# Zehong-Ma/MagCache

Measured on NVIDIA H100. Metric: denoising_steps_per_sec, higher is better.
Workload: dtype bf16

## Files before the change

magcache_b200/csrc/attn_wgmma.cu:

```cuda
#include <cstdlib>

#include "common.cuh"
#include "ptx.cuh"
#include "tma_host.cuh"

#ifndef MC_ATTN_EMU_DEFAULT
#define MC_ATTN_EMU_DEFAULT 0
#endif

namespace mc {

constexpr int kHD = 128;
constexpr int kLongMinLk = 1024;

struct AttnParams {
  int Lq, Lk, heads;
  int q_blocks, full_units, tail_units, tail_split;
  float* part_o;
  float2* part_ml;
  float scale_log2;
  __nv_bfloat16* out;
  int64_t ldo;
  int tile_rot;
  const uint32_t* seg_flags;
  const uint32_t* seg_epoch;
  int seg_rows;
};

struct WorkItem {
  int q_block, head;
  int split, nsplit;
  int tail_unit;
};

__device__ __forceinline__ WorkItem work_item(const AttnParams& p) {
  WorkItem w;
  int c = blockIdx.x, unit;
  if (c < p.full_units) {
    unit = c, w.split = 0, w.nsplit = 1, w.tail_unit = 0;
  } else {
    c -= p.full_units;
    w.tail_unit = c / p.tail_split;
    w.split = c - w.tail_unit * p.tail_split;
    w.nsplit = p.tail_split;
    unit = p.full_units + w.tail_unit;
  }
  w.head = unit / p.q_blocks;
  w.q_block = unit - w.head * p.q_blocks;
  return w;
}

template <uint32_t EMU_MASK>
__device__ __forceinline__ float exp2_sel(float x, int group) {
  return ((EMU_MASK >> (group & 7)) & 1u) ? ptx::ex2_emul(x) : ptx::ex2_approx(x);
}

__device__ __forceinline__ void wait_segments(const AttnParams& p, int row0, int rows) {
  if (p.seg_flags == nullptr) return;
  const uint32_t want = *reinterpret_cast<const volatile uint32_t*>(p.seg_epoch);
  const int last = min(row0 + rows, p.Lk) - 1;
  const int s0 = row0 / p.seg_rows, s1 = last / p.seg_rows;
  for (int s = s0; s <= s1; ++s) {
    const uint32_t* f = p.seg_flags + s;
    const long long t0 = clock64();
    for (;;) {
      uint32_t v;
      asm volatile("ld.acquire.sys.global.u32 %0, [%1];" : "=r"(v) : "l"(f) : "memory");
      if (static_cast<int32_t>(v - want) >= 0) break;
      __nanosleep(100);
      if (clock64() - t0 > MC_MBAR_TIMEOUT_CYCLES) {
        MC_DIAG("attention: key segment %d never arrived (flag %u, epoch %u)\n", s, v, want);
        __trap();
      }
    }
  }
  asm volatile("fence.proxy.async;" ::: "memory");
}

namespace ak {
constexpr int kBQ = 128;
constexpr int kQBytes = kBQ * kHD * 2;
constexpr int kThreads = 384;
constexpr int kProducerRegs = 24, kConsumerRegs = 240;
template <int BKV>
struct Layout {
  static constexpr int kKBytes = BKV * kHD * 2;
  static constexpr int kVBytes = BKV * kHD * 2;
  static constexpr int kOffK = kQBytes;
  static constexpr int kOffV = kOffK + 2 * kKBytes;
  static constexpr int kOffBar = kOffV + 2 * kVBytes;
  static constexpr int kSmem = kOffBar + 128;
};
}

template <int BKV, uint32_t EMU_MASK>
__global__ void __launch_bounds__(ak::kThreads, 1)
    attn_kernel(const __grid_constant__ CUtensorMap tmap_q, const __grid_constant__ CUtensorMap tmap_k,
                const __grid_constant__ CUtensorMap tmap_v, const AttnParams p) {
  using namespace ak;
  using L = Layout<BKV>;
  extern __shared__ __align__(1024) uint8_t smem[];
  uint64_t* bars = reinterpret_cast<uint64_t*>(smem + L::kOffBar);
  uint64_t* q_full = bars + 0;
  uint64_t* k_full = bars + 1;
  uint64_t* k_empty = bars + 3;
  uint64_t* v_full = bars + 5;
  uint64_t* v_empty = bars + 7;

  const int warp = threadIdx.x >> 5, lane = threadIdx.x & 31;
  const WorkItem wi = work_item(p);
  const int q0 = wi.q_block * kBQ;
  const int head = wi.head;
  const int total_tiles = (p.Lk + BKV - 1) / BKV;
  const int per_split = (total_tiles + wi.nsplit - 1) / wi.nsplit;
  const int t0 = wi.split * per_split;
  const int n_tiles = min(per_split, total_tiles - t0);
  auto tile_of = [&](int j) {
    int t = p.tile_rot + t0 + j;
    return t >= total_tiles ? t - total_tiles : t;
  };

  if (threadIdx.x == 0) {
    if ((ptx::smem_u32(smem) & 1023u) != 0) {
      MC_DIAG("attn_kernel: dynamic smem base not 1024-aligned\n");
      __trap();
    }
    ptx::prefetch_tmap(&tmap_q);
    ptx::prefetch_tmap(&tmap_k);
    ptx::prefetch_tmap(&tmap_v);
    ptx::mbar_init(q_full, 1);
    for (int s = 0; s < 2; ++s) {
      ptx::mbar_init(&k_full[s], 1);
      ptx::mbar_init(&k_empty[s], 8);
      ptx::mbar_init(&v_full[s], 1);
      ptx::mbar_init(&v_empty[s], 8);
    }
    ptx::fence_mbar_init();
  }
  __syncthreads();

  if (warp < 4) {
    ptx::setmaxnreg_dec<kProducerRegs>();
    if (warp == 0) {
      if (ptx::elect_one()) {
        ptx::mbar_expect_tx(q_full, kQBytes);
        ptx::tma_load_2d(smem, &tmap_q, q_full, head * kHD, q0);
        ptx::tma_load_2d(smem + kQBytes / 2, &tmap_q, q_full, head * kHD + 64, q0);
      }
      __syncwarp();
      for (int j = 0; j < n_tiles; ++j) {
        const int s = j & 1;
        const uint32_t ph = (j >> 1) & 1;
        const int kv0 = tile_of(j) * BKV;
        if (p.seg_flags != nullptr) {
          if (lane == 0) wait_segments(p, kv0, BKV);
          __syncwarp();
        }
        ptx::mbar_wait(&k_empty[s], ph ^ 1);
        if (ptx::elect_one()) {
          ptx::mbar_expect_tx(&k_full[s], L::kKBytes);
          ptx::tma_load_2d(smem + L::kOffK + s * L::kKBytes, &tmap_k, &k_full[s], head * kHD, kv0);
          ptx::tma_load_2d(smem + L::kOffK + s * L::kKBytes + L::kKBytes / 2, &tmap_k, &k_full[s], head * kHD + 64, kv0);
        }
        __syncwarp();
        ptx::mbar_wait(&v_empty[s], ph ^ 1);
        if (ptx::elect_one()) {
          ptx::mbar_expect_tx(&v_full[s], L::kVBytes);
          ptx::tma_load_2d(smem + L::kOffV + s * L::kVBytes, &tmap_v, &v_full[s], head * kHD, kv0);
          ptx::tma_load_2d(smem + L::kOffV + s * L::kVBytes + L::kVBytes / 2, &tmap_v, &v_full[s], head * kHD + 64, kv0);
        }
        __syncwarp();
      }
    }
  } else {
    ptx::setmaxnreg_inc<kConsumerRegs>();
    const int wg = (warp >> 2) - 1;
    const int r = wg * 64 + (warp & 3) * 16 + (lane >> 2);
    const int cq = 2 * (lane & 3);
    const uint32_t q_base = ptx::smem_u32(smem) + wg * (64 * 128);
    const uint32_t k_base = ptx::smem_u32(smem + L::kOffK), v_base = ptx::smem_u32(smem + L::kOffV);
    int j_ragged = -1;
    if (p.Lk % BKV != 0) {
      int jr = total_tiles - 1 - p.tile_rot - t0;
      if (jr < 0) jr += total_tiles;
      if (jr < n_tiles) j_ragged = jr;
    }
    float o[kHD / 2];
#pragma unroll
    for (int i = 0; i < kHD / 2; ++i) o[i] = 0.f;
    float m0 = -INFINITY, m1 = -INFINITY, l0 = 0.f, l1 = 0.f;
    bool timed_out = false;
    ptx::mbar_wait_or_flag(q_full, 0, timed_out);

    constexpr uint32_t kTurnThreads = 256;
    const uint32_t bar_own = 1 + wg, bar_other = 2 - wg;
    auto turn_begin = [&] { ptx::named_bar_sync(bar_own, kTurnThreads); };
    auto turn_end = [&] { ptx::named_bar_arrive(bar_other, kTurnThreads); };
    if (wg == 0) ptx::named_bar_arrive(bar_own, kTurnThreads);

    float sc[BKV / 2];
    uint32_t pa[BKV / 16][4];
    const int valid = p.Lk - (total_tiles - 1) * BKV;
    auto issue_s = [&](int j) {
      const int s = j & 1;
      ptx::wgmma_fence();
#pragma unroll
      for (int kk = 0; kk < kHD / 16; ++kk) {
        const uint64_t da = ptx::gmma_desc_sw128_kmajor(q_base + (kk >> 2) * (kQBytes / 2)) + 2 * (kk & 3);
        const uint64_t db = ptx::gmma_desc_sw128_kmajor(k_base + s * L::kKBytes + (kk >> 2) * (L::kKBytes / 2)) + 2 * (kk & 3);
        if constexpr (BKV == 128) {
          ptx::wgmma_m64n128k16_ss(sc, da, db, kk != 0 ? 1u : 0u);
        } else {
          ptx::wgmma_m64n64k16_ss(sc, da, db, kk != 0 ? 1u : 0u);
        }
      }
      ptx::wgmma_commit();
    };
    auto issue_pv = [&](int j) {
      const int s = j & 1;
      ptx::fence_regs(o);
      ptx::wgmma_fence();
      const uint64_t dv = ptx::gmma_desc_sw128_mnmajor(v_base + s * L::kVBytes, BKV * 128);
#pragma unroll
      for (int kk = 0; kk < BKV / 16; ++kk)
        ptx::wgmma_m64n128k16_rs_tb(o, pa[kk], dv + static_cast<uint64_t>(kk * (2048 / 16)), 1u);
      ptx::wgmma_commit();
    };
    auto softmax = [&](int j, float& f0, float& f1) {
      ptx::fence_regs(sc);
      __syncwarp();
      if (lane == 0) ptx::mbar_arrive(&k_empty[j & 1]);
      if (j == j_ragged) {
#pragma unroll
        for (int i = 0; i < BKV / 8; ++i)
#pragma unroll
          for (int e = 0; e < 4; ++e)
            if (8 * i + cq + (e & 1) >= valid) sc[4 * i + e] = -INFINITY;
      }
      float mx0 = -INFINITY, mx1 = -INFINITY;
#pragma unroll
      for (int i = 0; i < BKV / 8; ++i) {
        mx0 = fmaxf(mx0, fmaxf(sc[4 * i], sc[4 * i + 1]));
        mx1 = fmaxf(mx1, fmaxf(sc[4 * i + 2], sc[4 * i + 3]));
      }
#pragma unroll
      for (int off = 1; off <= 2; off <<= 1) {
        mx0 = fmaxf(mx0, __shfl_xor_sync(0xffffffffu, mx0, off));
        mx1 = fmaxf(mx1, __shfl_xor_sync(0xffffffffu, mx1, off));
      }
      const float mn0 = fmaxf(m0, mx0 * p.scale_log2), mn1 = fmaxf(m1, mx1 * p.scale_log2);
      f0 = ptx::ex2_approx(m0 - mn0), f1 = ptx::ex2_approx(m1 - mn1);
      m0 = mn0, m1 = mn1;
      l0 *= f0, l1 *= f1;
#pragma unroll
      for (int i = 0; i < BKV / 8; ++i) {
        sc[4 * i] = exp2_sel<EMU_MASK>(fmaf(sc[4 * i], p.scale_log2, -m0), i);
        sc[4 * i + 1] = exp2_sel<EMU_MASK>(fmaf(sc[4 * i + 1], p.scale_log2, -m0), i);
        sc[4 * i + 2] = exp2_sel<EMU_MASK>(fmaf(sc[4 * i + 2], p.scale_log2, -m1), i);
        sc[4 * i + 3] = exp2_sel<EMU_MASK>(fmaf(sc[4 * i + 3], p.scale_log2, -m1), i);
        l0 += sc[4 * i] + sc[4 * i + 1];
        l1 += sc[4 * i + 2] + sc[4 * i + 3];
      }
    };
    auto pack_p = [&] {
#pragma unroll
      for (int i = 0; i < BKV / 8; ++i) {
        pa[i >> 1][(i & 1) * 2] = pack_bf16x2(sc[4 * i], sc[4 * i + 1]);
        pa[i >> 1][(i & 1) * 2 + 1] = pack_bf16x2(sc[4 * i + 2], sc[4 * i + 3]);
      }
    };
    auto release_v = [&](int j) {
      ptx::fence_regs(o);
      __syncwarp();
      if (lane == 0) ptx::mbar_arrive(&v_empty[j & 1]);
    };
    auto rescale_o = [&](float f0, float f1) {
#pragma unroll
      for (int i = 0; i < kHD / 8; ++i) {
        o[4 * i] *= f0, o[4 * i + 1] *= f0;
        o[4 * i + 2] *= f1, o[4 * i + 3] *= f1;
      }
    };
    {
      ptx::mbar_wait_or_flag(&k_full[0], 0, timed_out);
      turn_begin();
      issue_s(0);
      turn_end();
      ptx::wgmma_wait<0>();
      float f0, f1;
      softmax(0, f0, f1);
      rescale_o(f0, f1);
      pack_p();
    }
    for (int j = 1; j < n_tiles; ++j) {
      ptx::mbar_wait_or_flag(&k_full[j & 1], (j >> 1) & 1, timed_out);
      ptx::mbar_wait_or_flag(&v_full[(j - 1) & 1], ((j - 1) >> 1) & 1, timed_out);
      turn_begin();
      issue_s(j);
      issue_pv(j - 1);
      turn_end();
      ptx::wgmma_wait<1>();
      float f0, f1;
      softmax(j, f0, f1);
      ptx::wgmma_wait<0>();
      release_v(j - 1);
      rescale_o(f0, f1);
      pack_p();
    }
    {
      const int j = n_tiles - 1;
      ptx::mbar_wait_or_flag(&v_full[j & 1], (j >> 1) & 1, timed_out);
      turn_begin();
      issue_pv(j);
      if (wg == 0) turn_end();
      ptx::wgmma_wait<0>();
      release_v(j);
    }
    if (timed_out) __trap();

#pragma unroll
    for (int off = 1; off <= 2; off <<= 1) {
      l0 += __shfl_xor_sync(0xffffffffu, l0, off);
      l1 += __shfl_xor_sync(0xffffffffu, l1, off);
    }
    const bool partial = wi.nsplit > 1;
#pragma unroll
    for (int h = 0; h < 2; ++h) {
      const float inv_l = 1.0f / (h ? l1 : l0);
      const int rt = r + 8 * h;
      const int row = q0 + rt;
      if (row >= p.Lq) continue;
      if (partial) {
        const int64_t prow = (static_cast<int64_t>(wi.split) * p.tail_units + wi.tail_unit) * kBQ + rt;
        if ((lane & 3) == 0) p.part_ml[prow] = make_float2(h ? m1 : m0, h ? l1 : l0);
        float* dst = p.part_o + prow * kHD + cq;
#pragma unroll
        for (int i = 0; i < kHD / 8; ++i)
          *reinterpret_cast<float2*>(dst + 8 * i) = make_float2(o[4 * i + 2 * h] * inv_l, o[4 * i + 2 * h + 1] * inv_l);
      } else {
        __nv_bfloat16* dst = p.out + static_cast<int64_t>(row) * p.ldo + head * kHD + cq;
#pragma unroll
        for (int i = 0; i < kHD / 8; ++i)
          *reinterpret_cast<uint32_t*>(dst + 8 * i) = pack_bf16x2(o[4 * i + 2 * h] * inv_l, o[4 * i + 2 * h + 1] * inv_l);
      }
    }
  }
}

__global__ void __launch_bounds__(256) attn_combine_kernel(const float* __restrict__ part_o, const float2* __restrict__ part_ml, int nsplit,
                                                           int tail_units, int full_units, int q_blocks, int rows_per_cta, int Lq,
                                                           __nv_bfloat16* __restrict__ out, int64_t ldo) {
  constexpr int kGroups = kHD / 8;
  const int64_t total = static_cast<int64_t>(tail_units) * rows_per_cta * kGroups;
  const int64_t split_stride = static_cast<int64_t>(tail_units) * rows_per_cta;
  for (int64_t i = static_cast<int64_t>(blockIdx.x) * blockDim.x + threadIdx.x; i < total; i += static_cast<int64_t>(gridDim.x) * blockDim.x) {
    const int64_t prow = i / kGroups;
    const int g = static_cast<int>(i - prow * kGroups);
    const int tu = static_cast<int>(prow / rows_per_cta), r = static_cast<int>(prow - static_cast<int64_t>(tu) * rows_per_cta);
    const int unit = full_units + tu;
    const int head = unit / q_blocks, row = (unit - head * q_blocks) * rows_per_cta + r;
    if (row >= Lq) continue;
    float mmax = -INFINITY;
    for (int s = 0; s < nsplit; ++s) mmax = fmaxf(mmax, part_ml[s * split_stride + prow].x);
    float acc[8] = {0.f, 0.f, 0.f, 0.f, 0.f, 0.f, 0.f, 0.f};
    float wsum = 0.f;
    for (int s = 0; s < nsplit; ++s) {
      const float2 ml = part_ml[s * split_stride + prow];
      const float w = ml.y * ptx::ex2_approx(ml.x - mmax);
      wsum += w;
      float v[8];
      ptx::ld_nc_v8_f32(part_o + (s * split_stride + prow) * kHD + g * 8, v);
#pragma unroll
      for (int j = 0; j < 8; ++j) acc[j] = fmaf(w, v[j], acc[j]);
    }
    const float inv = 1.0f / wsum;
#pragma unroll
    for (int j = 0; j < 8; ++j) acc[j] *= inv;
    *reinterpret_cast<uint4*>(out + static_cast<int64_t>(row) * ldo + head * kHD + g * 8) = pack_bf16x8(acc);
  }
}

struct AttnPlan {
  bool long_kernel;
  int q_blocks, kv_tile, total_tiles, rows_per_cta;
  int full_units, tail_units, tail_split;
  size_t ws_bytes;
  int grid() const { return full_units + tail_units * tail_split; }
};

static int env_int(const char* name, int lo, int hi, int dflt) {
  const char* e = getenv(name);
  if (!e || !*e) return dflt;
  const int v = atoi(e);
  return (v < lo || v > hi) ? dflt : v;
}

static AttnPlan plan_attention(int Lq, int Lk, int heads, bool need_long = false) {
  AttnPlan pl;
  const int forced_splits = env_int("MC_ATTN_SPLITS", 1, 16, 0);
  const int kernel_sel = env_int("MC_ATTN_KERNEL", 0, 2, 0);
  pl.long_kernel = need_long || kernel_sel == 2 || (kernel_sel == 0 && Lk >= kLongMinLk);
  pl.rows_per_cta = ak::kBQ;
  pl.kv_tile = pl.long_kernel ? 128 : 64;
  pl.q_blocks = (Lq + pl.rows_per_cta - 1) / pl.rows_per_cta;
  pl.total_tiles = (Lk + pl.kv_tile - 1) / pl.kv_tile;
  const int64_t units = static_cast<int64_t>(pl.q_blocks) * heads;
  const int slots = num_sms();
  const int min_tiles_per_split = pl.long_kernel ? 4 : 8;
  int full = static_cast<int>(units), tail = 0, split = 1;
  if (forced_splits > 0) {
    if (forced_splits > 1) full = 0, tail = static_cast<int>(units), split = forced_splits;
  } else {
    const int rem = static_cast<int>(units % slots);
    const int by_tiles = pl.total_tiles / min_tiles_per_split;
    int f = rem > 0 ? slots / rem : 1;
    if (f > 8) f = 8;
    if (f > by_tiles) f = by_tiles;
    if (f >= 2) full = static_cast<int>(units) - rem, tail = rem, split = f;
  }
  if (split > pl.total_tiles) split = pl.total_tiles;
  if (split > 1) {
    const int per = (pl.total_tiles + split - 1) / split;
    split = (pl.total_tiles + per - 1) / per;
  }
  if (split <= 1) full = static_cast<int>(units), tail = 0, split = 1;
  pl.full_units = full, pl.tail_units = tail, pl.tail_split = split;
  pl.ws_bytes = tail > 0 ? static_cast<size_t>(split) * tail * pl.rows_per_cta * (kHD * sizeof(float) + sizeof(float2)) : 0;
  return pl;
}

}

extern "C" int32_t mc_attn_workspace_bytes(int32_t Lq, int32_t Lk, int32_t heads, int64_t* bytes_out) {
  MC_CHECK_ARG(bytes_out != nullptr && Lq >= 1 && Lk >= 1 && heads >= 1, "mc_attn_workspace_bytes: bad arguments");
  const size_t a = mc::plan_attention(Lq, Lk, heads, false).ws_bytes, b = mc::plan_attention(Lq, Lk, heads, true).ws_bytes;
  *bytes_out = static_cast<int64_t>(a > b ? a : b);
  return MC_OK;
}

extern "C" int32_t mc_attn_fwd_ex(const void* q, int64_t ldq, const void* k, int64_t ldk, const void* v, int64_t ldv, void* out,
                                  int64_t ldo, int32_t Lq, int32_t Lk, int32_t heads, float scale, void* workspace,
                                  int64_t workspace_bytes, int32_t first_key_row, const uint32_t* seg_flags, const uint32_t* seg_epoch,
                                  int32_t seg_rows, void* stream) {
  MC_CHECK_ARG(q && k && v && out, "mc_attn_fwd: null pointer");
  MC_CHECK_ARG(Lq >= 1 && Lk >= 1 && heads >= 1, "mc_attn_fwd: Lq=%d Lk=%d heads=%d", Lq, Lk, heads);
  const int64_t width = static_cast<int64_t>(heads) * mc::kHD;
  MC_CHECK_ARG(ldq >= width && ldk >= width && ldo >= width && ldv >= width, "mc_attn_fwd: leading dimensions too small");
  MC_CHECK_ARG(ldq % 8 == 0 && ldk % 8 == 0 && ldv % 8 == 0 && ldo % 8 == 0, "mc_attn_fwd: leading dimensions must be multiples of 8");
  MC_CHECK_ARG(mc::aligned16(q) && mc::aligned16(k) && mc::aligned16(v) && mc::aligned16(out), "mc_attn_fwd: pointers must be 16-byte aligned");
  MC_CHECK_ARG(first_key_row >= 0 && first_key_row < Lk, "mc_attn_fwd: first_key_row=%d outside [0, %d)", first_key_row, Lk);
  MC_CHECK_ARG(seg_flags == nullptr || (seg_rows >= 1 && seg_epoch != nullptr), "mc_attn_fwd: seg_rows=%d / null epoch", seg_rows);
  const mc::AttnPlan pl = mc::plan_attention(Lq, Lk, heads, first_key_row != 0 || seg_flags != nullptr);
  MC_CHECK_ARG(static_cast<int64_t>(pl.q_blocks) * heads * 8 < INT32_MAX, "mc_attn_fwd: grid too large");
  if (pl.tail_units > 0) {
    MC_CHECK_ARG(workspace != nullptr && workspace_bytes >= static_cast<int64_t>(pl.ws_bytes) && (reinterpret_cast<uintptr_t>(workspace) & 31u) == 0,
                 "mc_attn_fwd: split-KV needs a 32-byte aligned workspace of %lld bytes (mc_attn_workspace_bytes), got %lld",
                 static_cast<long long>(pl.ws_bytes), static_cast<long long>(workspace_bytes));
  }
  const int q_box = mc::ak::kBQ;
  CUtensorMap tq, tk, tv;
  int32_t rc = mc::make_tmap_bf16_2d(&tq, q, static_cast<uint64_t>(Lq), static_cast<uint64_t>(width), static_cast<uint64_t>(ldq), q_box, 64);
  if (rc) return rc;
  rc = mc::make_tmap_bf16_2d(&tk, k, static_cast<uint64_t>(Lk), static_cast<uint64_t>(width), static_cast<uint64_t>(ldk), pl.kv_tile, 64);
  if (rc) return rc;
  rc = mc::make_tmap_bf16_2d(&tv, v, static_cast<uint64_t>(Lk), static_cast<uint64_t>(width), static_cast<uint64_t>(ldv), pl.kv_tile, 64);
  if (rc) return rc;

  float* part_o = static_cast<float*>(workspace);
  const size_t part_rows = static_cast<size_t>(pl.tail_split) * pl.tail_units * pl.rows_per_cta;
  float2* part_ml = pl.tail_units > 0 ? reinterpret_cast<float2*>(part_o + part_rows * mc::kHD) : nullptr;
  mc::AttnParams p{};
  p.Lq = Lq, p.Lk = Lk, p.heads = heads;
  p.q_blocks = pl.q_blocks, p.full_units = pl.full_units, p.tail_units = pl.tail_units, p.tail_split = pl.tail_split;
  p.part_o = pl.tail_units > 0 ? part_o : nullptr, p.part_ml = part_ml;
  p.scale_log2 = scale * 1.4426950408889634f;
  p.out = static_cast<__nv_bfloat16*>(out), p.ldo = ldo;
  p.tile_rot = ((first_key_row + pl.kv_tile - 1) / pl.kv_tile) % pl.total_tiles;
  p.seg_flags = seg_flags, p.seg_epoch = seg_epoch, p.seg_rows = seg_rows > 0 ? seg_rows : Lk;

  dim3 grid(pl.grid(), 1, 1);
  cudaStream_t st = static_cast<cudaStream_t>(stream);
  if (pl.long_kernel) {
    static mc::PerDeviceOnce once[4];
    const int emu = mc::env_int("MC_ATTN_EMU", 0, 4, MC_ATTN_EMU_DEFAULT);
#define MC_LAUNCH_LONG(MASK, IDX)                                                                                                    \
  do {                                                                                                                               \
    rc = mc::set_max_smem_once(mc::attn_kernel<128, MASK>, mc::ak::Layout<128>::kSmem, once[IDX], "cudaFuncSetAttribute(attn smem)"); \
    if (rc) return rc;                                                                                                               \
    mc::attn_kernel<128, MASK><<<grid, mc::ak::kThreads, mc::ak::Layout<128>::kSmem, st>>>(tq, tk, tv, p);                           \
  } while (0)
    switch (emu) {
      case 2: MC_LAUNCH_LONG(0x88u, 1); break;
      case 3: MC_LAUNCH_LONG(0x92u, 2); break;
      case 4: MC_LAUNCH_LONG(0xAAu, 3); break;
      default: MC_LAUNCH_LONG(0x00u, 0); break;
    }
#undef MC_LAUNCH_LONG
  } else {
    static mc::PerDeviceOnce once;
    rc = mc::set_max_smem_once(mc::attn_kernel<64, 0u>, mc::ak::Layout<64>::kSmem, once, "cudaFuncSetAttribute(attn smem)");
    if (rc) return rc;
    mc::attn_kernel<64, 0u><<<grid, mc::ak::kThreads, mc::ak::Layout<64>::kSmem, st>>>(tq, tk, tv, p);
  }
  MC_CHECK_LAUNCH("attn_kernel launch");
  if (pl.tail_units > 0) {
    const int64_t total = static_cast<int64_t>(pl.tail_units) * pl.rows_per_cta * (mc::kHD / 8);
    const int64_t want = (total + 255) / 256, cap = static_cast<int64_t>(mc::num_sms()) * 8;
    mc::attn_combine_kernel<<<static_cast<int>(want < cap ? want : cap), 256, 0, st>>>(
        p.part_o, p.part_ml, pl.tail_split, pl.tail_units, pl.full_units, pl.q_blocks, pl.rows_per_cta, Lq, static_cast<__nv_bfloat16*>(out), ldo);
    MC_CHECK_LAUNCH("attn_combine_kernel launch");
  }
  return MC_OK;
}

extern "C" int32_t mc_attn_fwd(const void* q, int64_t ldq, const void* k, int64_t ldk, const void* v, int64_t ldv, void* out,
                               int64_t ldo, int32_t Lq, int32_t Lk, int32_t heads, float scale, void* workspace,
                               int64_t workspace_bytes, void* stream) {
  return mc_attn_fwd_ex(q, ldq, k, ldk, v, ldv, out, ldo, Lq, Lk, heads, scale, workspace, workspace_bytes, 0, nullptr, nullptr, 0, stream);
}
```

Before: 1.661.

## Pair attention CTAs in 2-CTA clusters sharing K/V tiles via TMA multicast

```diff
diff --git a/magcache_b200/csrc/attn_wgmma.cu b/magcache_b200/csrc/attn_wgmma.cu
--- a/magcache_b200/csrc/attn_wgmma.cu
+++ b/magcache_b200/csrc/attn_wgmma.cu
@@ -33,16 +33,20 @@
   int tail_unit;
 };
 
+template <bool PAIR>
 __device__ __forceinline__ WorkItem work_item(const AttnParams& p) {
   WorkItem w;
-  int c = blockIdx.x, unit;
-  if (c < p.full_units) {
-    unit = c, w.split = 0, w.nsplit = 1, w.tail_unit = 0;
+  constexpr int kW = PAIR ? 2 : 1;
+  const int rank = PAIR ? static_cast<int>(ptx::cluster_ctarank()) : 0;
+  int c = PAIR ? static_cast<int>(blockIdx.x >> 1) : static_cast<int>(blockIdx.x), unit;
+  if (c < p.full_units / kW) {
+    unit = kW * c + rank, w.split = 0, w.nsplit = 1, w.tail_unit = 0;
   } else {
-    c -= p.full_units;
-    w.tail_unit = c / p.tail_split;
-    w.split = c - w.tail_unit * p.tail_split;
+    c -= p.full_units / kW;
+    const int item = c / p.tail_split;
+    w.split = c - item * p.tail_split;
     w.nsplit = p.tail_split;
+    w.tail_unit = kW * item + rank;
     unit = p.full_units + w.tail_unit;
   }
   w.head = unit / p.q_blocks;
@@ -82,6 +86,7 @@
 constexpr int kQBytes = kBQ * kHD * 2;
 constexpr int kThreads = 384;
 constexpr int kProducerRegs = 24, kConsumerRegs = 240;
+constexpr int kPairCluster = 2;
 template <int BKV>
 struct Layout {
   static constexpr int kKBytes = BKV * kHD * 2;
@@ -93,12 +98,14 @@
 };
 }
 
-template <int BKV, uint32_t EMU_MASK>
+template <int BKV, uint32_t EMU_MASK, bool PAIR>
 __global__ void __launch_bounds__(ak::kThreads, 1)
     attn_kernel(const __grid_constant__ CUtensorMap tmap_q, const __grid_constant__ CUtensorMap tmap_k,
                 const __grid_constant__ CUtensorMap tmap_v, const AttnParams p) {
   using namespace ak;
   using L = Layout<BKV>;
+  static_assert(!PAIR || BKV == 128, "only the 128-key kernel is paired");
+  constexpr uint32_t kCtas = PAIR ? kPairCluster : 1;
   extern __shared__ __align__(1024) uint8_t smem[];
   uint64_t* bars = reinterpret_cast<uint64_t*>(smem + L::kOffBar);
   uint64_t* q_full = bars + 0;
@@ -108,7 +115,7 @@
   uint64_t* v_empty = bars + 7;
 
   const int warp = threadIdx.x >> 5, lane = threadIdx.x & 31;
-  const WorkItem wi = work_item(p);
+  const WorkItem wi = work_item<PAIR>(p);
   const int q0 = wi.q_block * kBQ;
   const int head = wi.head;
   const int total_tiles = (p.Lk + BKV - 1) / BKV;
@@ -131,13 +138,18 @@
     ptx::mbar_init(q_full, 1);
     for (int s = 0; s < 2; ++s) {
       ptx::mbar_init(&k_full[s], 1);
-      ptx::mbar_init(&k_empty[s], 8);
+      ptx::mbar_init(&k_empty[s], 8 * kCtas);
       ptx::mbar_init(&v_full[s], 1);
-      ptx::mbar_init(&v_empty[s], 8);
+      ptx::mbar_init(&v_empty[s], 8 * kCtas);
     }
     ptx::fence_mbar_init();
   }
-  __syncthreads();
+  if constexpr (PAIR) {
+    ptx::cluster_arrive();
+    ptx::cluster_wait();
+  } else {
+    __syncthreads();
+  }
 
   if (warp < 4) {
     ptx::setmaxnreg_dec<kProducerRegs>();
@@ -148,26 +160,38 @@
         ptx::tma_load_2d(smem + kQBytes / 2, &tmap_q, q_full, head * kHD + 64, q0);
       }
       __syncwarp();
+      const uint32_t rank = PAIR ? ptx::cluster_ctarank() : 0u;
       for (int j = 0; j < n_tiles; ++j) {
         const int s = j & 1;
         const uint32_t ph = (j >> 1) & 1;
         const int kv0 = tile_of(j) * BKV;
+        const int row0 = kv0 + static_cast<int>(rank) * (BKV / kCtas);
+        const uint32_t part = rank * (L::kKBytes / 2 / kCtas);
+        auto load = [&](uint8_t* dst, const CUtensorMap* tmap, uint64_t* bar, int c0) {
+          if constexpr (PAIR) {
+            ptx::tma_load_2d_multicast(dst, tmap, bar, c0, row0, static_cast<uint16_t>((1u << kCtas) - 1));
+          } else {
+            ptx::tma_load_2d(dst, tmap, bar, c0, row0);
+          }
+        };
         if (p.seg_flags != nullptr) {
-          if (lane == 0) wait_segments(p, kv0, BKV);
+          if (lane == 0) wait_segments(p, row0, BKV / kCtas);
           __syncwarp();
         }
         ptx::mbar_wait(&k_empty[s], ph ^ 1);
         if (ptx::elect_one()) {
+          uint8_t* dst = smem + L::kOffK + s * L::kKBytes + part;
           ptx::mbar_expect_tx(&k_full[s], L::kKBytes);
-          ptx::tma_load_2d(smem + L::kOffK + s * L::kKBytes, &tmap_k, &k_full[s], head * kHD, kv0);
-          ptx::tma_load_2d(smem + L::kOffK + s * L::kKBytes + L::kKBytes / 2, &tmap_k, &k_full[s], head * kHD + 64, kv0);
+          load(dst, &tmap_k, &k_full[s], head * kHD);
+          load(dst + L::kKBytes / 2, &tmap_k, &k_full[s], head * kHD + 64);
         }
         __syncwarp();
         ptx::mbar_wait(&v_empty[s], ph ^ 1);
         if (ptx::elect_one()) {
+          uint8_t* dst = smem + L::kOffV + s * L::kVBytes + part;
           ptx::mbar_expect_tx(&v_full[s], L::kVBytes);
-          ptx::tma_load_2d(smem + L::kOffV + s * L::kVBytes, &tmap_v, &v_full[s], head * kHD, kv0);
-          ptx::tma_load_2d(smem + L::kOffV + s * L::kVBytes + L::kVBytes / 2, &tmap_v, &v_full[s], head * kHD + 64, kv0);
+          load(dst, &tmap_v, &v_full[s], head * kHD);
+          load(dst + L::kVBytes / 2, &tmap_v, &v_full[s], head * kHD + 64);
         }
         __syncwarp();
       }
@@ -226,10 +250,18 @@
         ptx::wgmma_m64n128k16_rs_tb(o, pa[kk], dv + static_cast<uint64_t>(kk * (2048 / 16)), 1u);
       ptx::wgmma_commit();
     };
+    auto release = [&](uint64_t* bar) {
+      if (lane != 0) return;
+      if constexpr (PAIR) {
+        for (uint32_t c = 0; c < kCtas; ++c) ptx::mbar_arrive_cluster(bar, c);
+      } else {
+        ptx::mbar_arrive(bar);
+      }
+    };
     auto softmax = [&](int j, float& f0, float& f1) {
       ptx::fence_regs(sc);
       __syncwarp();
-      if (lane == 0) ptx::mbar_arrive(&k_empty[j & 1]);
+      release(&k_empty[j & 1]);
       if (j == j_ragged) {
 #pragma unroll
         for (int i = 0; i < BKV / 8; ++i)
@@ -272,9 +304,10 @@
     auto release_v = [&](int j) {
       ptx::fence_regs(o);
       __syncwarp();
-      if (lane == 0) ptx::mbar_arrive(&v_empty[j & 1]);
+      release(&v_empty[j & 1]);
     };
     auto rescale_o = [&](float f0, float f1) {
+      if (!__any_sync(0xffffffffu, f0 != 1.f || f1 != 1.f)) return;
 #pragma unroll
       for (int i = 0; i < kHD / 8; ++i) {
         o[4 * i] *= f0, o[4 * i + 1] *= f0;
@@ -289,7 +322,6 @@
       ptx::wgmma_wait<0>();
       float f0, f1;
       softmax(0, f0, f1);
-      rescale_o(f0, f1);
       pack_p();
     }
     for (int j = 1; j < n_tiles; ++j) {
@@ -344,6 +376,10 @@
           *reinterpret_cast<uint32_t*>(dst + 8 * i) = pack_bf16x2(o[4 * i + 2 * h] * inv_l, o[4 * i + 2 * h + 1] * inv_l);
       }
     }
+  }
+  if constexpr (PAIR) {
+    ptx::cluster_arrive();
+    ptx::cluster_wait();
   }
 }
 
@@ -381,7 +417,7 @@
 }
 
 struct AttnPlan {
-  bool long_kernel;
+  bool long_kernel, paired;
   int q_blocks, kv_tile, total_tiles, rows_per_cta;
   int full_units, tail_units, tail_split;
   size_t ws_bytes;
@@ -395,28 +431,79 @@
   return (v < lo || v > hi) ? dflt : v;
 }
 
-static AttnPlan plan_attention(int Lq, int Lk, int heads, bool need_long = false) {
+static PerDeviceOnce g_attn_smem_once[2][4][2];
+
+template <uint32_t MASK>
+static int emu_index() {
+  return MASK == 0x88u ? 1 : MASK == 0x92u ? 2 : MASK == 0xAAu ? 3 : 0;
+}
+template <int BKV, uint32_t MASK, bool PAIR>
+static int32_t attn_set_smem() {
+  return set_max_smem_once(attn_kernel<BKV, MASK, PAIR>, ak::Layout<BKV>::kSmem, g_attn_smem_once[BKV == 128][emu_index<MASK>()][PAIR],
+                           "cudaFuncSetAttribute(attn smem)");
+}
+
+static int32_t attn_pair_clusters(int* out) {
+  static int cached[kMaxDevices] = {};
+  const int d = current_device();
+  if (cached[d] > 0) {
+    *out = cached[d];
+    return MC_OK;
+  }
+  int devices = 0;
+  if (cudaGetDeviceCount(&devices) != cudaSuccess || devices < 1) {
+    cudaGetLastError();
+    *out = num_sms() / ak::kPairCluster;
+    return MC_OK;
+  }
+  int32_t rc = attn_set_smem<128, 0u, true>();
+  if (rc) return rc;
+  cudaLaunchAttribute attr[1];
+  attr[0].id = cudaLaunchAttributeClusterDimension;
+  attr[0].val.clusterDim.x = ak::kPairCluster, attr[0].val.clusterDim.y = 1, attr[0].val.clusterDim.z = 1;
+  cudaLaunchConfig_t cfg = {};
+  cfg.gridDim = dim3(ak::kPairCluster * num_sms(), 1, 1);
+  cfg.blockDim = dim3(ak::kThreads, 1, 1);
+  cfg.dynamicSmemBytes = ak::Layout<128>::kSmem;
+  cfg.attrs = attr, cfg.numAttrs = 1;
+  int n = 0;
+  const cudaError_t e = cudaOccupancyMaxActiveClusters(&n, attn_kernel<128, 0u, true>, &cfg);
+  if (e != cudaSuccess) return cuda_fail(e, "cudaOccupancyMaxActiveClusters(attn)");
+  if (n < 1) {
+    set_error("attn_kernel: no cluster of %d CTAs with %d B of shared memory fits on this device", ak::kPairCluster, ak::Layout<128>::kSmem);
+    return MC_ERR_CUDA;
+  }
+  cached[d] = n;
+  *out = n;
+  return MC_OK;
+}
+
+static AttnPlan plan_attention(int Lq, int Lk, int heads, bool need_long, int pair_clusters) {
   AttnPlan pl;
   const int forced_splits = env_int("MC_ATTN_SPLITS", 1, 16, 0);
   const int kernel_sel = env_int("MC_ATTN_KERNEL", 0, 2, 0);
   pl.long_kernel = need_long || kernel_sel == 2 || (kernel_sel == 0 && Lk >= kLongMinLk);
+  pl.paired = pl.long_kernel && pair_clusters > 0;
   pl.rows_per_cta = ak::kBQ;
   pl.kv_tile = pl.long_kernel ? 128 : 64;
   pl.q_blocks = (Lq + pl.rows_per_cta - 1) / pl.rows_per_cta;
+  if (pl.paired) pl.q_blocks += pl.q_blocks & 1;
   pl.total_tiles = (Lk + pl.kv_tile - 1) / pl.kv_tile;
+  const int w = pl.paired ? ak::kPairCluster : 1;
   const int64_t units = static_cast<int64_t>(pl.q_blocks) * heads;
-  const int slots = num_sms();
+  const int64_t items = units / w;
+  const int slots = pl.paired ? pair_clusters : num_sms();
   const int min_tiles_per_split = pl.long_kernel ? 4 : 8;
   int full = static_cast<int>(units), tail = 0, split = 1;
   if (forced_splits > 0) {
     if (forced_splits > 1) full = 0, tail = static_cast<int>(units), split = forced_splits;
   } else {
-    const int rem = static_cast<int>(units % slots);
+    const int rem = static_cast<int>(items % slots);
     const int by_tiles = pl.total_tiles / min_tiles_per_split;
     int f = rem > 0 ? slots / rem : 1;
     if (f > 8) f = 8;
     if (f > by_tiles) f = by_tiles;
-    if (f >= 2) full = static_cast<int>(units) - rem, tail = rem, split = f;
+    if (f >= 2) full = static_cast<int>(units) - rem * w, tail = rem * w, split = f;
   }
   if (split > pl.total_tiles) split = pl.total_tiles;
   if (split > 1) {
@@ -429,12 +516,50 @@
   return pl;
 }
 
+static int32_t attn_pair_slots(int* out) {
+  *out = 0;
+  if (env_int("MC_ATTN_PAIR", 0, 1, 1) == 0) return MC_OK;
+  return attn_pair_clusters(out);
+}
+
+template <int BKV, uint32_t MASK, bool PAIR>
+static int32_t launch_attn(const CUtensorMap& tq, const CUtensorMap& tk, const CUtensorMap& tv, const AttnParams& p, int grid,
+                           cudaStream_t st) {
+  int32_t rc = attn_set_smem<BKV, MASK, PAIR>();
+  if (rc) return rc;
+  if constexpr (PAIR) {
+    cudaLaunchAttribute attr[1];
+    attr[0].id = cudaLaunchAttributeClusterDimension;
+    attr[0].val.clusterDim.x = ak::kPairCluster, attr[0].val.clusterDim.y = 1, attr[0].val.clusterDim.z = 1;
+    cudaLaunchConfig_t cfg = {};
+    cfg.gridDim = dim3(grid, 1, 1);
+    cfg.blockDim = dim3(ak::kThreads, 1, 1);
+    cfg.dynamicSmemBytes = ak::Layout<BKV>::kSmem;
+    cfg.stream = st;
+    cfg.attrs = attr, cfg.numAttrs = 1;
+    const cudaError_t e = cudaLaunchKernelEx(&cfg, attn_kernel<BKV, MASK, PAIR>, tq, tk, tv, p);
+    if (e != cudaSuccess) return cuda_fail(e, "attn_kernel launch (paired)");
+  } else {
+    attn_kernel<BKV, MASK, PAIR><<<grid, ak::kThreads, ak::Layout<BKV>::kSmem, st>>>(tq, tk, tv, p);
+  }
+  MC_CHECK_LAUNCH("attn_kernel launch");
+  return MC_OK;
+}
+
 }
 
 extern "C" int32_t mc_attn_workspace_bytes(int32_t Lq, int32_t Lk, int32_t heads, int64_t* bytes_out) {
   MC_CHECK_ARG(bytes_out != nullptr && Lq >= 1 && Lk >= 1 && heads >= 1, "mc_attn_workspace_bytes: bad arguments");
-  const size_t a = mc::plan_attention(Lq, Lk, heads, false).ws_bytes, b = mc::plan_attention(Lq, Lk, heads, true).ws_bytes;
-  *bytes_out = static_cast<int64_t>(a > b ? a : b);
+  int clusters = 0;
+  const int32_t rc = mc::attn_pair_clusters(&clusters);
+  if (rc) return rc;
+  size_t most = 0;
+  for (int need_long = 0; need_long < 2; ++need_long)
+    for (int paired = 0; paired < 2; ++paired) {
+      const size_t b = mc::plan_attention(Lq, Lk, heads, need_long != 0, paired ? clusters : 0).ws_bytes;
+      if (b > most) most = b;
+    }
+  *bytes_out = static_cast<int64_t>(most);
   return MC_OK;
 }
 
@@ -450,7 +575,10 @@
   MC_CHECK_ARG(mc::aligned16(q) && mc::aligned16(k) && mc::aligned16(v) && mc::aligned16(out), "mc_attn_fwd: pointers must be 16-byte aligned");
   MC_CHECK_ARG(first_key_row >= 0 && first_key_row < Lk, "mc_attn_fwd: first_key_row=%d outside [0, %d)", first_key_row, Lk);
   MC_CHECK_ARG(seg_flags == nullptr || (seg_rows >= 1 && seg_epoch != nullptr), "mc_attn_fwd: seg_rows=%d / null epoch", seg_rows);
-  const mc::AttnPlan pl = mc::plan_attention(Lq, Lk, heads, first_key_row != 0 || seg_flags != nullptr);
+  int pair_clusters = 0;
+  int32_t rc = mc::attn_pair_slots(&pair_clusters);
+  if (rc) return rc;
+  const mc::AttnPlan pl = mc::plan_attention(Lq, Lk, heads, first_key_row != 0 || seg_flags != nullptr, pair_clusters);
   MC_CHECK_ARG(static_cast<int64_t>(pl.q_blocks) * heads * 8 < INT32_MAX, "mc_attn_fwd: grid too large");
   if (pl.tail_units > 0) {
     MC_CHECK_ARG(workspace != nullptr && workspace_bytes >= static_cast<int64_t>(pl.ws_bytes) && (reinterpret_cast<uintptr_t>(workspace) & 31u) == 0,
@@ -458,12 +586,13 @@
                  static_cast<long long>(pl.ws_bytes), static_cast<long long>(workspace_bytes));
   }
   const int q_box = mc::ak::kBQ;
+  const int kv_box = pl.paired ? pl.kv_tile / mc::ak::kPairCluster : pl.kv_tile;
   CUtensorMap tq, tk, tv;
-  int32_t rc = mc::make_tmap_bf16_2d(&tq, q, static_cast<uint64_t>(Lq), static_cast<uint64_t>(width), static_cast<uint64_t>(ldq), q_box, 64);
-  if (rc) return rc;
-  rc = mc::make_tmap_bf16_2d(&tk, k, static_cast<uint64_t>(Lk), static_cast<uint64_t>(width), static_cast<uint64_t>(ldk), pl.kv_tile, 64);
-  if (rc) return rc;
-  rc = mc::make_tmap_bf16_2d(&tv, v, static_cast<uint64_t>(Lk), static_cast<uint64_t>(width), static_cast<uint64_t>(ldv), pl.kv_tile, 64);
+  rc = mc::make_tmap_bf16_2d(&tq, q, static_cast<uint64_t>(Lq), static_cast<uint64_t>(width), static_cast<uint64_t>(ldq), q_box, 64);
+  if (rc) return rc;
+  rc = mc::make_tmap_bf16_2d(&tk, k, static_cast<uint64_t>(Lk), static_cast<uint64_t>(width), static_cast<uint64_t>(ldk), kv_box, 64);
+  if (rc) return rc;
+  rc = mc::make_tmap_bf16_2d(&tv, v, static_cast<uint64_t>(Lk), static_cast<uint64_t>(width), static_cast<uint64_t>(ldv), kv_box, 64);
   if (rc) return rc;
 
   float* part_o = static_cast<float*>(workspace);
@@ -478,31 +607,23 @@
   p.tile_rot = ((first_key_row + pl.kv_tile - 1) / pl.kv_tile) % pl.total_tiles;
   p.seg_flags = seg_flags, p.seg_epoch = seg_epoch, p.seg_rows = seg_rows > 0 ? seg_rows : Lk;
 
-  dim3 grid(pl.grid(), 1, 1);
+  const int grid = pl.grid();
   cudaStream_t st = static_cast<cudaStream_t>(stream);
   if (pl.long_kernel) {
-    static mc::PerDeviceOnce once[4];
     const int emu = mc::env_int("MC_ATTN_EMU", 0, 4, MC_ATTN_EMU_DEFAULT);
-#define MC_LAUNCH_LONG(MASK, IDX)                                                                                                    \
-  do {                                                                                                                               \
-    rc = mc::set_max_smem_once(mc::attn_kernel<128, MASK>, mc::ak::Layout<128>::kSmem, once[IDX], "cudaFuncSetAttribute(attn smem)"); \
-    if (rc) return rc;                                                                                                               \
-    mc::attn_kernel<128, MASK><<<grid, mc::ak::kThreads, mc::ak::Layout<128>::kSmem, st>>>(tq, tk, tv, p);                           \
-  } while (0)
+#define MC_LAUNCH_LONG(MASK) \
+  (pl.paired ? mc::launch_attn<128, MASK, true>(tq, tk, tv, p, grid, st) : mc::launch_attn<128, MASK, false>(tq, tk, tv, p, grid, st))
     switch (emu) {
-      case 2: MC_LAUNCH_LONG(0x88u, 1); break;
-      case 3: MC_LAUNCH_LONG(0x92u, 2); break;
-      case 4: MC_LAUNCH_LONG(0xAAu, 3); break;
-      default: MC_LAUNCH_LONG(0x00u, 0); break;
+      case 2: rc = MC_LAUNCH_LONG(0x88u); break;
+      case 3: rc = MC_LAUNCH_LONG(0x92u); break;
+      case 4: rc = MC_LAUNCH_LONG(0xAAu); break;
+      default: rc = MC_LAUNCH_LONG(0x00u); break;
     }
 #undef MC_LAUNCH_LONG
   } else {
-    static mc::PerDeviceOnce once;
-    rc = mc::set_max_smem_once(mc::attn_kernel<64, 0u>, mc::ak::Layout<64>::kSmem, once, "cudaFuncSetAttribute(attn smem)");
-    if (rc) return rc;
-    mc::attn_kernel<64, 0u><<<grid, mc::ak::kThreads, mc::ak::Layout<64>::kSmem, st>>>(tq, tk, tv, p);
-  }
-  MC_CHECK_LAUNCH("attn_kernel launch");
+    rc = mc::launch_attn<64, 0u, false>(tq, tk, tv, p, grid, st);
+  }
+  if (rc) return rc;
   if (pl.tail_units > 0) {
     const int64_t total = static_cast<int64_t>(pl.tail_units) * pl.rows_per_cta * (mc::kHD / 8);
     const int64_t want = (total + 255) / 256, cap = static_cast<int64_t>(mc::num_sms()) * 8;
```

After: 1.705 (median of 6 runs). 2.6% higher.
